# spacetelescope/subpixal

Measured on AMD Instinct MI355X. Metric: cutout cross-correlations/sec (64x64 px, upsample=10), higher is better.
Workload: dtype f32; 1 GPU; BASELINE.json configs[1]: 100000 64x64 Gaussian-spot cutout pairs per GPU, upsample=10, inputs resident in HBM; pairs_per_gpu=100000, tile=64, upsample=10, cc_type=CC, refine=default, parallelism=batch sharded over 1 GPU(s); gather of (dx,dy) to rank 0

## Files before the change

### subpixal_amd/csrc/spx_kernels.h

```cpp
#pragma once

namespace spx {

using rt::f32x2;
using rt::f32x4;
typedef f32x2 cf;

constexpr int kThreads = 256;

SPX_DEVICE int fresh_tid() { return rt::launder_lane(rt::thread_id()); }

enum { ST_OK = 0, ST_EDGE = 1, ST_NOMAX = 2, ST_OUTSIDE = 3, ST_WINDOW = 4, ST_FEWPTS = 5, ST_NONFINITE = 6, ST_SHAPE = 7 };
constexpr int kNoIndex = 0x7fffffff;
enum { CC_PLAIN = 0, CC_NCC = 1, CC_ZNCC = 2 };

constexpr int kNumPhases = 20;
template <int DBG> struct PhaseClock {
    unsigned long long last;
    unsigned long long acc[DBG == 100 ? kNumPhases : 1];
    SPX_DEVICE void start() {
        if constexpr (DBG == 100) {
            for (int i = 0; i < kNumPhases; ++i) acc[i] = 0;
            last = rt::clock_stamp();
        }
// ... 48 lines not shown
#pragma unroll
        for (int y = 0; y < 8; ++y) t[y] = v[y][x];
        fft8<DIR>(t);
#pragma unroll
        for (int y = 0; y < 8; ++y) v[y][x] = t[y];
    }
}
template <int DIR> SPX_DEVICE void fft8_x(cf (&v)[8][8]) {
#pragma unroll
    for (int y = 0; y < 8; ++y) fft8<DIR>(v[y]);
}

#ifndef SPX_CMUL_BATCH
#define SPX_CMUL_BATCH 1
#endif
template <bool CONJ> SPX_DEVICE void mul_row(cf (&v)[8][8], int y, cf w) {
    if constexpr (SPX_CMUL_BATCH) {
        rt::cmul8_ip<CONJ>(v[y][0], v[y][1], v[y][2], v[y][3], v[y][4], v[y][5], v[y][6], v[y][7], w);
    } else {
#pragma unroll
        for (int x = 0; x < 8; ++x) { if (CONJ) rt::cmulc_ip(v[y][x], w); else rt::cmul_ip(v[y][x], w); }
    }
}
template <bool CONJ> SPX_DEVICE void mul_col(cf (&v)[8][8], int x, cf w) {
    if constexpr (SPX_CMUL_BATCH) {
        rt::cmul8_ip<CONJ>(v[0][x], v[1][x], v[2][x], v[3][x], v[4][x], v[5][x], v[6][x], v[7][x], w);
    } else {
#pragma unroll
        for (int y = 0; y < 8; ++y) { if (CONJ) rt::cmulc_ip(v[y][x], w); else rt::cmul_ip(v[y][x], w); }
    }
}

template <int XS> SPX_DEVICE void transpose_tile(cf (&v)[8][8], float* xch, int lane) {
#pragma unroll
    for (int part = 0; part < 2; ++part) {
#pragma unroll
        for (int r = 0; r < 64; ++r)
            xch[r * XS + lane] = part ? v[r >> 3][r & 7].y : v[r >> 3][r & 7].x;
        rt::wave_sync();
#pragma unroll
        for (int r = 0; r < 64; ++r) {
            const float t = xch[lane * XS + r];
            if (part) v[r >> 3][r & 7].y = t; else v[r >> 3][r & 7].x = t;
        }
        rt::wave_sync();
    }
}

template <int XS> SPX_DEVICE void transpose_tile_v(cf (&v)[8][8], float* xch, int lane) {
#pragma unroll
    for (int part = 0; part < 2; ++part) {
#pragma unroll
        for (int r = 0; r < 64; ++r)
            xch[r * XS + lane] = part ? v[r >> 3][r & 7].y : v[r >> 3][r & 7].x;
        rt::wave_sync();
#pragma unroll
        for (int r = 0; r < 64; ++r) {
            const float t = rt::lds_read_f32(xch + lane * XS + r);
            if (part) v[r >> 3][r & 7].y = t; else v[r >> 3][r & 7].x = t;
        }
        rt::wave_sync();
    }
}

template <int XS> SPX_DEVICE void transpose_tile_w(cf (&v)[8][8], float* xch, int lane) {
    static_assert(XS >= 68 && (XS & 3) == 0, "32 complex slots per row plus the conflict padding");
    cf* buf = reinterpret_cast<cf*>(xch);
    cf t[64];
#pragma unroll
    for (int h = 0; h < 2; ++h) {
        if ((lane >> 5) == h) {
#pragma unroll
            for (int r = 0; r < 64; ++r) buf[r * (XS / 2) + (lane & 31)] = v[r >> 3][r & 7];
        }
        rt::wave_sync();
        const f32x4* row = reinterpret_cast<const f32x4*>(buf + lane * (XS / 2));
#pragma unroll
        for (int j = 0; j < 16; ++j) {
            const f32x4 q = row[j];
            t[32 * h + 2 * j] = cf{q[0], q[1]};
            t[32 * h + 2 * j + 1] = cf{q[2], q[3]};
        }
        rt::wave_sync();
    }
#pragma unroll
    for (int r = 0; r < 64; ++r) v[r >> 3][r & 7] = t[r];
}

#ifndef SPX_TRANSPOSE_VARIANT
#define SPX_TRANSPOSE_VARIANT 0
#endif
template <int XS> SPX_DEVICE void transpose_tile_sel(cf (&v)[8][8], float* xch, int lane) {
    if constexpr (SPX_TRANSPOSE_VARIANT == 1) transpose_tile_v<XS>(v, xch, lane);
    else if constexpr (SPX_TRANSPOSE_VARIANT == 2) transpose_tile_w<XS>(v, xch, lane);
    else transpose_tile<XS>(v, xch, lane);
}

SPX_DEVICE int plane_elem(int row, int col) { return row * 64 + (col ^ ((row & 7) << 3)); }
SPX_DEVICE int plane_slot(int n) { return n ^ (((n >> 4) & 7) << 1); }

template <int XS> SPX_DEVICE void transpose_tile_cplx(cf (&v)[8][8], float* xch, int lane) {
    constexpr int RS = 66;
    static_assert(32 * RS * 2 <= 64 * XS, "half a tile must fit the wave's exchange buffer");
    cf* buf = reinterpret_cast<cf*>(xch);
    cf t[64];
#pragma unroll
    for (int h = 0; h < 2; ++h) {
#pragma unroll
        for (int r = 0; r < 32; ++r) buf[r * RS + lane] = v[(32 * h + r) >> 3][(32 * h + r) & 7];
        rt::wave_sync();
        if ((lane >> 5) == h) {
            const f32x4* row = reinterpret_cast<const f32x4*>(buf + (lane & 31) * RS);
#pragma unroll
            for (int j = 0; j < 32; ++j) {
                const f32x4 q = row[j];
                t[2 * j] = cf{q[0], q[1]};
                t[2 * j + 1] = cf{q[2], q[3]};
            }
        }
        rt::wave_sync();
    }
#pragma unroll
    for (int r = 0; r < 64; ++r) v[r >> 3][r & 7] = t[r];
}

template <int C> struct Lds {
    static constexpr int P = 64 * C;
    static constexpr int T = 32 * C;
    static constexpr int NCLS = C * C;
    static constexpr int ZS = 72;
    static constexpr int XS = 68;
    static constexpr int PS = 64;
    static constexpr int TW_OFF = 0;
    static constexpr int SCR_OFF = TW_OFF + P * 8;
    static constexpr int R_OFF = SCR_OFF + 1024;
    static constexpr int ZBUF_BYTES = 2 * 64 * ZS * 4;
    static constexpr int XCH_WAVE_BYTES = 64 * XS * 4;
    static constexpr int XCH_BYTES = NCLS * XCH_WAVE_BYTES;
    static constexpr int PLANE_STRIDE_BYTES = XCH_WAVE_BYTES;
    static constexpr int FB_OFF = R_OFF + XCH_BYTES;
    static constexpr int cmax(int a, int b) { return a > b ? a : b; }
    static constexpr int fb_count(int W) { return W <= 16 ? NCLS : 1; }
    static constexpr int total(int W) {
        return cmax(R_OFF + cmax(ZBUF_BYTES, XCH_BYTES), FB_OFF + fb_count(W) * W * W * 4);
    }
};

constexpr int SCR_RED_F = 0;
constexpr int SCR_INT = 64;
constexpr int SCR_RED_D = 128;
constexpr int SCR_FIT = 256;
constexpr int SCR_STAT = 512;
constexpr int SCR_RED_D6 = 576;

SPX_DEVICE double wave_sum(double v) {
#pragma unroll
    for (int m = 32; m >= 1; m >>= 1) v += rt::shfl_xor(v, m);
    return v;
}

template <int NV> SPX_DEVICE void block_sum(unsigned char* lds_scr, double (&v)[NV]) {
    static_assert(NV <= 4 || NV == 6, "scratch slots exist for up to 4 values, or exactly 6");
    constexpr int ST = NV <= 4 ? 4 : 6;
    const int tid = rt::thread_id();
    double* part = reinterpret_cast<double*>(lds_scr + (NV <= 4 ? SCR_RED_D : SCR_RED_D6));
#pragma unroll
    for (int i = 0; i < NV; ++i) v[i] = wave_sum(v[i]);
    if ((tid & 63) == 0) {
#pragma unroll
        for (int i = 0; i < NV; ++i) part[(tid >> 6) * ST + i] = v[i];
    }
    rt::block_sync_lds();
#pragma unroll
    for (int i = 0; i < NV; ++i) {
        double s = 0.0;
        for (int w = 0; w < kThreads / 64; ++w) s += part[w * ST + i];
        v[i] = s;
    }
    rt::block_sync_lds();
}

SPX_DEVICE void block_sum2f(unsigned char* lds_scr, float& a, float& b) {
    const int tid = rt::thread_id();
#pragma unroll
    for (int m = 32; m >= 1; m >>= 1) {
        a += rt::shfl_xor(a, m);
        b += rt::shfl_xor(b, m);
    }
    float* part = reinterpret_cast<float*>(lds_scr + SCR_STAT);
    if ((tid & 63) == 0) { part[2 * (tid >> 6)] = a; part[2 * (tid >> 6) + 1] = b; }
    rt::block_sync_lds();
    a = (part[0] + part[2]) + (part[4] + part[6]);
    b = (part[1] + part[3]) + (part[5] + part[7]);
}

SPX_DEVICE bool better(float v, int i, float bv, int bi) {
    return (v > bv) || (v == bv && i < bi);
}
SPX_DEVICE float nan_as_inf(float v) { return v != v ? __builtin_inff() : v; }

template <int STEP> SPX_DEVICE void argmax_step(float& v, int& idx) {
    const float ov = rt::row_xchg<STEP>(v);
    const int oi = rt::row_xchg<STEP>(idx);
    if (better(ov, oi, v, idx)) { v = ov; idx = oi; }
}
SPX_DEVICE void wave_argmax(float& v, int& idx) {
    argmax_step<0>(v, idx);
    argmax_step<1>(v, idx);
    argmax_step<2>(v, idx);
    argmax_step<3>(v, idx);
    float bv = rt::read_lane(v, 0);
    int bi = rt::read_lane(idx, 0);
#pragma unroll
    for (int r = 1; r < 4; ++r) {
        const float ov = rt::read_lane(v, 16 * r);
        const int oi = rt::read_lane(idx, 16 * r);
        if (better(ov, oi, bv, bi)) { bv = ov; bi = oi; }
    }
    v = bv;
    idx = bi;
}

SPX_DEVICE void block_argmax(unsigned char* lds_scr, float& v, int& idx, int slot) {
    const int tid = rt::thread_id();
    wave_argmax(v, idx);
    float* rf = reinterpret_cast<float*>(lds_scr + SCR_RED_F) + 8 * slot;
    int* ri = reinterpret_cast<int*>(lds_scr + SCR_RED_F) + 8 * slot + 4;
    if ((tid & 63) == 0) { rf[tid >> 6] = v; ri[tid >> 6] = idx; }
    rt::block_sync_lds();
    v = rf[0];
    idx = ri[0];
    for (int w = 1; w < kThreads / 64; ++w)
        if (better(rf[w], ri[w], v, idx)) { v = rf[w]; idx = ri[w]; }
}

struct PeakResult {
    double x, y;
    int status;
};

SPX_DEVICE PeakResult quad_fit_finish(double s0, double sx, double sy, double sxy, double sxx,
                                      double syy, int x1, int y1, int imax, int jmax, int nx,
                                      int ny) {
    const double c10 = sx * (1.0 / 50.0), c01 = sy * (1.0 / 50.0), c11 = sxy * (1.0 / 100.0);
    const double c20 = (sxx - 2.0 * s0) * (1.0 / 70.0), c02 = (syy - 2.0 * s0) * (1.0 / 70.0);
    PeakResult r;
    const double det = 4.0 * c02 * c20 - c11 * c11;
    if (det <= 0.0 || ((c20 > 0.0 && c02 >= 0.0) || (c20 >= 0.0 && c02 > 0.0))) {
        r.x = x1 + 2.5;
        r.y = y1 + 2.5;
        r.status = ST_NOMAX;
        return r;
    }
    const double inv_det = 1.0 / det;
    const double xm = (x1 + 2) + (c01 * c11 - 2.0 * c02 * c10) * inv_det;
    const double ym = (y1 + 2) + (c10 * c11 - 2.0 * c01 * c20) * inv_det;
    if (xm > 0.0 && xm < nx - 1.0 && ym > 0.0 && ym < ny - 1.0) {
        r.x = xm;
        r.y = ym;
        r.status = ST_OK;
    } else {
        r.x = (double)imax;
        r.y = (double)jmax;
        r.status = ST_OUTSIDE;
    }
    return r;
}

SPX_DEVICE PeakResult quad_fit_5x5(const double* d, int x1, int y1, int imax, int jmax,
                                   int nx, int ny) {
    double s0 = 0, sx = 0, sy = 0, sxy = 0, sxx = 0, syy = 0;
    for (int j = 0; j < 5; ++j) {
        for (int i = 0; i < 5; ++i) {
            double v = d[j * 5 + i];
            double x = (double)(i - 2), y = (double)(j - 2);
            s0 += v;
            sx += x * v;
            sy += y * v;
            sxy += x * y * v;
            sxx += x * x * v;
            syy += y * y * v;
        }
    }
    return quad_fit_finish(s0, sx, sy, sxy, sxx, syy, x1, y1, imax, jmax, nx, ny);
}

SPX_DEVICE PeakResult quad_fit_wave(float v, int lane, int x1, int y1, int imax, int jmax,
                                    int nx, int ny) {
    lane = rt::launder_lane(lane);
    const int j = lane < 6 ? lane : 0;
    const int px = (j == 1 || j == 3) ? 1 : (j == 4 ? 2 : 0);
    const int py = (j == 2 || j == 3) ? 1 : (j == 5 ? 2 : 0);
    double xw[5], yw[5];
#pragma unroll
    for (int i = 0; i < 5; ++i) {
        const double c = (double)(i - 2);
        xw[i] = px == 0 ? 1.0 : (px == 1 ? c : c * c);
        yw[i] = py == 0 ? 1.0 : (py == 1 ? c : c * c);
    }
    double s = 0.0;
#pragma unroll
    for (int y = 0; y < 5; ++y) {
        double row = 0.0;
#pragma unroll
        for (int x = 0; x < 5; ++x) row += xw[x] * (double)rt::read_lane(v, 5 * y + x);
        s += yw[y] * row;
    }
    const double s0 = rt::read_lane(s, 0), sx = rt::read_lane(s, 1), sy = rt::read_lane(s, 2);
    const double sxy = rt::read_lane(s, 3), sxx = rt::read_lane(s, 4), syy = rt::read_lane(s, 5);
    return quad_fit_finish(s0, sx, sy, sxy, sxx, syy, x1, y1, imax, jmax, nx, ny);
}

SPX_DEVICE int64_t first_item(int64_t b, int64_t nwg) {
#ifdef SPX_LINEAR_WALK
    return b;
#endif
    if (nwg & 63) return b;
    const int64_t x = b & 7, j = b >> 3;
    return ((j >> 3) << 6) + (x << 3) + (j & 7);
}

template <int C> SPX_DEVICE void load_twiddles(unsigned char* lds, const cf* __restrict__ tw_g) {
    typedef Lds<C> L;
    cf* tw = reinterpret_cast<cf*>(lds + L::TW_OFF);
    for (int i = rt::thread_id(); i < L::P; i += kThreads) tw[i] = tw_g[i];
    rt::block_sync_lds();
}

SPX_DEVICE float warm_next_pair(const float* __restrict__ ref, const float* __restrict__ img) {
    const int tid = rt::thread_id();
    const float* p = (tid < 128) ? ref + tid * 32 : img + (tid - 128) * 32;
    return *p;
}

template <typename T> struct NormStatsT {
    T im_mean, im_rstd, ref_mean, ref_rstd;
    int active;
};

template <typename T> struct Quad { T v[4]; };
struct __attribute__((packed, aligned(4))) PackedF4 { float v[4]; };
struct __attribute__((packed, aligned(8))) PackedD2 { double v[2]; };
struct __attribute__((packed, aligned(4))) PackedF2 { float v[2]; };
SPX_DEVICE Quad<float> load_quad(const float* p) {
    const PackedF4 t = *reinterpret_cast<const PackedF4*>(p);
    return Quad<float>{{t.v[0], t.v[1], t.v[2], t.v[3]}};
}
SPX_DEVICE Quad<double> load_quad(const double* p) {
    const PackedD2 a = *reinterpret_cast<const PackedD2*>(p);
    const PackedD2 b = *reinterpret_cast<const PackedD2*>(p + 2);
    return Quad<double>{{a.v[0], a.v[1], b.v[0], b.v[1]}};
}
template <typename T> SPX_DEVICE float norm_im(T m, const NormStatsT<T>& ns) {
    if (m != (T)0) { m = m - ns.im_mean; m = m * ns.im_rstd; }
    return (float)m;
}
template <typename T> SPX_DEVICE float norm_ref(T r, const NormStatsT<T>& ns) {
    r = r - ns.ref_mean;
    return (float)(r * ns.ref_rstd);
}

template <typename TIn> struct ChunkLoad {
    Quad<TIn> r, t;
    int s;
    bool in;
};
template <typename TIn, bool NARROW, bool NX4 = false>
SPX_DEVICE ChunkLoad<TIn> chunk_issue(const TIn* __restrict__ ref, const TIn* __restrict__ img,
                                      int ny, int nx, int y, int x) {
    ChunkLoad<TIn> c;
    c.in = y < ny && x < nx;
    const int yy = y < ny ? y : ny - 1;
    if (NARROW) {
        c.s = 4 - nx;
        const TIn* rrow = ref + (int64_t)yy * nx;
        const TIn* mrow = img + (int64_t)(ny - 1 - yy) * nx;
#pragma unroll
        for (int k = 0; k < 4; ++k) {
            c.r.v[k] = k >= c.s ? rrow[k - c.s] : (TIn)0;
            c.t.v[k] = k < nx ? mrow[k] : (TIn)0;
        }
        c.in = c.in && x == 0;
        return c;
    }
    const int xx = x < nx ? x : 0;
    int s = xx + 4 - nx;
    s = (NX4 || s < 0) ? 0 : s;
    c.s = s;
    c.r = load_quad(ref + (int64_t)yy * nx + (xx - s));
    c.t = load_quad(img + (int64_t)(ny - 1 - yy) * nx + (nx - 4 - xx + s));
    return c;
}
template <typename T> SPX_DEVICE T quad_pick(const Quad<T>& q, int k) {
    const T lo = k & 1 ? q.v[1] : q.v[0], hi = k & 1 ? q.v[3] : q.v[2];
    return k & 2 ? hi : lo;
}
template <typename TIn>
SPX_DEVICE void chunk_unpack(const ChunkLoad<TIn>& c, const NormStatsT<TIn>& ns, float (&re)[4],
                             float (&im)[4]) {
#pragma unroll
    for (int e = 0; e < 4; ++e) {
        const bool ok = c.in && e + c.s < 4;
        const TIn ri = quad_pick(c.r, (e + c.s) & 3);
        const TIn mi = quad_pick(c.t, (3 - c.s - e) & 3);
        float r = (float)ri, m = (float)mi;
        if (ns.active) {
            m = norm_im(mi, ns);
            r = norm_ref(ri, ns);
        }
        re[e] = ok ? r : 0.0f;
        im[e] = ok ? m : 0.0f;
    }
}

template <int C, bool FOLD> struct StageGeom {
    static constexpr int ZS = FOLD ? 88 : 96;
    static constexpr int ROWS = FOLD ? 88 : 64;
    static constexpr int CHUNKS = (FOLD ? 88 : 64) / 4;
    static constexpr int PS12 = 12;
    static_assert(2 * ROWS * ZS * 4 <= Lds<C>::XCH_BYTES, "the staged input must fit the exchange region it shares");
    static SPX_DEVICE int perm(int q, int e) { return (4 * (q & 1) + e) * PS12 + (q >> 1); }
};

template <int C, bool FOLD = false, typename TIn = float, bool NARROW = false, bool NX4 = false>
SPX_DEVICE void stage_pair_rows(unsigned char* lds, const TIn* __restrict__ ref,
                           const TIn* __restrict__ img, int ny, int nx,
                           const NormStatsT<TIn>& ns, float (&ssq)[2]) {
    typedef Lds<C> L;
    typedef StageGeom<C, FOLD> G;
    float sr = 0.0f, sm = 0.0f;
    const int tid = fresh_tid();
    float* zre = reinterpret_cast<float*>(lds + L::R_OFF);
    float* zim = zre + G::ROWS * G::ZS;
    const bool aligned = ((reinterpret_cast<uintptr_t>(ref) | reinterpret_cast<uintptr_t>(img)) & 15) == 0;
    if constexpr (!FOLD && sizeof(TIn) == 4) if (ny == 64 && nx == 64 && aligned) {
        const f32x4* r4 = reinterpret_cast<const f32x4*>(ref);
        const f32x4* m4 = reinterpret_cast<const f32x4*>(img);
#pragma unroll
        for (int i = 0; i < 4; ++i) {
            const int idx = tid + i * kThreads;
            const int y = idx >> 4;
            f32x4 r = r4[idx];
            const f32x4 t = m4[(63 - y) * 16 + (15 - (idx & 15))];
            f32x4 m = f32x4{t[3], t[2], t[1], t[0]};
            if (ns.active) {
#pragma unroll
                for (int e = 0; e < 4; ++e) {
                    m[e] = norm_im(m[e], ns);
                    r[e] = norm_ref(r[e], ns);
                }
            }
#pragma unroll
            for (int e = 0; e < 4; ++e) {
                zre[y * G::ZS + G::perm(idx & 15, e)] = r[e];
                zim[y * G::ZS + G::perm(idx & 15, e)] = m[e];
                sr += r[e] * r[e];
                sm += m[e] * m[e];
            }
        }
        ssq[0] = sr;
        ssq[1] = sm;
        return;
    }
    constexpr int kIters = (G::ROWS * G::CHUNKS + kThreads - 1) / kThreads;
    ChunkLoad<TIn> ld[kIters];
#pragma unroll
    for (int i = 0; i < kIters; ++i) {
        const int idx = tid + i * kThreads;
        const int y = FOLD ? idx / G::CHUNKS : idx >> 4;
        const int x = (FOLD ? idx - y * G::CHUNKS : (idx & 15)) << 2;
        ld[i] = chunk_issue<TIn, NARROW, NX4>(ref, img, ny, nx, y, x);
    }
#pragma unroll
    for (int i = 0; i < kIters; ++i) {
        const int idx = tid + i * kThreads;
        if (FOLD && idx >= G::ROWS * G::CHUNKS) break;
        const int y = FOLD ? idx / G::CHUNKS : idx >> 4;
        const int x = (FOLD ? idx - y * G::CHUNKS : (idx & 15)) << 2;
        float rr[4], mm[4];
        chunk_unpack(ld[i], ns, rr, mm);
        if constexpr (FOLD) {
            *reinterpret_cast<f32x4*>(zre + y * G::ZS + x) = f32x4{rr[0], rr[1], rr[2], rr[3]};
            *reinterpret_cast<f32x4*>(zim + y * G::ZS + x) = f32x4{mm[0], mm[1], mm[2], mm[3]};
        } else {
#pragma unroll
            for (int e = 0; e < 4; ++e) {
                zre[y * G::ZS + G::perm(x >> 2, e)] = rr[e];
                zim[y * G::ZS + G::perm(x >> 2, e)] = mm[e];
            }
        }
#pragma unroll
        for (int e = 0; e < 4; ++e) { sr += rr[e] * rr[e]; sm += mm[e] * mm[e]; }
    }
    ssq[0] = sr;
    ssq[1] = sm;
}
template <int C, bool FOLD = false, typename TIn = float>
SPX_DEVICE void stage_pair(unsigned char* lds, const TIn* __restrict__ ref,
                           const TIn* __restrict__ img, int ny, int nx,
                           const NormStatsT<TIn>& ns, float (&ssq)[2]) {
    if (nx < 4) stage_pair_rows<C, FOLD, TIn, true>(lds, ref, img, ny, nx, ns, ssq);
    else if ((nx & 3) == 0) stage_pair_rows<C, FOLD, TIn, false, true>(lds, ref, img, ny, nx, ns, ssq);
    else stage_pair_rows<C, FOLD, TIn, false>(lds, ref, img, ny, nx, ns, ssq);
}

SPX_DEVICE float balance_from_ssq(float s0, float s1) {
    if (!(s0 > 0.0f) || !(s1 > 0.0f)) return 1.0f;
    const int e0 = (int)((__builtin_bit_cast(unsigned, s0) >> 23) & 0xffu);
    const int e1 = (int)((__builtin_bit_cast(unsigned, s1) >> 23) & 0xffu);
    int e = (e0 - e1) >> 1;
    e = e < -100 ? -100 : (e > 100 ? 100 : e);
    return __builtin_bit_cast(float, (unsigned)(127 + e) << 23);
}
SPX_DEVICE float balance_factor(unsigned char* lds_scr, float (&ssq)[2]) {
    block_sum2f(lds_scr, ssq[0], ssq[1]);
    return balance_from_ssq(ssq[0], ssq[1]);
}

SPX_DEVICE int plane_col(int row, int col) { return col ^ (((row & 1) << 4) | ((row & 2) << 2)); }

#ifndef SPX_DISP5_CPLXT
#define SPX_DISP5_CPLXT 0
#endif
#ifndef SPX_FUSED_TW
#define SPX_FUSED_TW 0
#endif
template <int K> SPX_DEVICE f32x2 quad_pair(f32x4 q) {
    if constexpr (K < 2) return f32x2{q[0], q[1]}; else return f32x2{q[2], q[3]};
}
template <int K, bool CONJ> SPX_DEVICE cf soa_cmul_k(f32x4 re4, f32x4 im4, cf w) {
    return rt::bcast_fma_rot<(K & 1), CONJ>(quad_pair<K>(im4), w, rt::bcast_mul<(K & 1), CONJ>(quad_pair<K>(re4), w));
}
template <bool CONJ> SPX_DEVICE cf soa_cmul(int k, f32x4 re4, f32x4 im4, cf w) {
    switch (k & 3) {
        case 0: return soa_cmul_k<0, CONJ>(re4, im4, w);
        case 1: return soa_cmul_k<1, CONJ>(re4, im4, w);
        case 2: return soa_cmul_k<2, CONJ>(re4, im4, w);
        default: return soa_cmul_k<3, CONJ>(re4, im4, w);
    }
}
template <int K> SPX_DEVICE cf soa_cmul2_k(f32x4 re4, f32x4 im4, cf w, cf bw) {
    return rt::bcast_fma_rot<(K & 1), false>(quad_pair<K>(im4), bw, rt::bcast_mul<(K & 1), false>(quad_pair<K>(re4), w));
}
SPX_DEVICE cf soa_cmul2(int k, f32x4 re4, f32x4 im4, cf w, cf bw) {
    switch (k & 3) {
        case 0: return soa_cmul2_k<0>(re4, im4, w, bw);
        case 1: return soa_cmul2_k<1>(re4, im4, w, bw);
        case 2: return soa_cmul2_k<2>(re4, im4, w, bw);
        default: return soa_cmul2_k<3>(re4, im4, w, bw);
    }
}

template <int XS, bool CONJ, bool W0_ONE>
SPX_DEVICE void transpose_tile_tw(cf (&v)[8][8], float* xch, int lane, const cf (&w)[8]) {
    f32x4 re4[16], im4[16];
#pragma unroll
    for (int part = 0; part < 2; ++part) {
#pragma unroll
        for (int r = 0; r < 64; ++r)
            xch[r * XS + lane] = part ? v[r >> 3][r & 7].y : v[r >> 3][r & 7].x;
        rt::wave_sync();
        const f32x4* row = reinterpret_cast<const f32x4*>(xch + lane * XS);
#pragma unroll
        for (int j = 0; j < 16; ++j) { if (part) im4[j] = row[j]; else re4[j] = row[j]; }
        rt::wave_sync();
    }
#pragma unroll
    for (int r = 0; r < 64; ++r) {
        const int b = r & 7;
        if (W0_ONE && b == 0) v[r >> 3][b] = cf{re4[r >> 2][r & 3], im4[r >> 2][r & 3]};
        else v[r >> 3][b] = soa_cmul<CONJ>(r, re4[r >> 2], im4[r >> 2], w[b]);
    }
}

template <typename G, int CY, int CX>
SPX_DEVICE void load_tile_class(cf (&v)[8][8], const float* zre, const float* zim, const cf* tw, float bal,
                                int l1, int l0) {
    constexpr int NK = 7 * (CY + CX) + 1;
    cf W[NK], BW[NK];
#pragma unroll
    for (int k = 1; k < NK; ++k) { W[k] = tw[8 * k]; BW[k] = cf{bal * W[k].x, bal * W[k].y}; }
#pragma unroll
    for (int y1 = 0; y1 < 8; ++y1) {
        const f32x4* pr = reinterpret_cast<const f32x4*>(zre + (l1 + 8 * y1) * G::ZS + l0 * G::PS12);
        const f32x4* pi = reinterpret_cast<const f32x4*>(zim + (l1 + 8 * y1) * G::ZS + l0 * G::PS12);
        const f32x4 r0 = pr[0], r1 = pr[1], i0 = pi[0], i1 = pi[1];
#pragma unroll
        for (int x1 = 0; x1 < 8; ++x1) {
            const int k = CY * y1 + CX * x1;
            const f32x4 rq = x1 < 4 ? r0 : r1, iq = x1 < 4 ? i0 : i1;
            if (k == 0) v[y1][x1] = cf{rq[x1 & 3], bal * iq[x1 & 3]};
            else v[y1][x1] = soa_cmul2(x1, rq, iq, W[k], BW[k]);
        }
    }
}

template <typename L, int CY, int CX>
SPX_DEVICE void store_plane_class(const cf (&v)[8][8], float* plane, const cf* tw, int l1, int l0) {
    constexpr int NK = 7 * (CY + CX) + 1;
    cf W[NK];
#pragma unroll
    for (int k = 1; k < NK; ++k) W[k] = tw[8 * k];
#pragma unroll
    for (int x1 = 0; x1 < 8; ++x1)
#pragma unroll
        for (int y1 = 0; y1 < 8; ++y1) {
            const cf a = v[y1][x1];
            const int k = CY * y1 + CX * x1;
            const int row = l1 + 8 * y1;
            plane[row * L::PS + plane_col(row, l0 + 8 * x1)] = k == 0 ? a.y : a.y * W[k].x - a.x * W[k].y;
        }
}
// ... 345 lines not shown
#pragma unroll
        for (int b = 0; b < WB; ++b)
#pragma unroll
            for (int i = 0; i < 4; ++i) {
                ft.ky[b][i] = kty[b * 64 * 4 + i];
                ft.kx[b][i] = ktx[b * 64 * 4 + i];
            }
    }
}

template <int C, int WB, typename R>
SPX_DEVICE void fine_window(unsigned char* lds, const FineTables<WB, R>& ft,
                            int ny, int nx, int qyc, int qxc, int rot = 0) {
    typedef Lds<C> L;
    typedef typename R::S S;
    typedef typename R::V4 V4;
    static_assert(C == 2, "");
    constexpr int W = 16 * WB;
    const int tid = fresh_tid();
    const int wave = ((tid >> 6) + rot) & (C * C - 1), lane = tid & 63;
    const int cy = wave / C, cx = wave % C;
    const int lk = lane >> 4, lj = lane & 15;
    const float* plane = reinterpret_cast<const float*>(lds + L::R_OFF + wave * L::PLANE_STRIDE_BYTES);
    float* fbuf = reinterpret_cast<float*>(lds + L::FB_OFF);
    const int lyc = conv_index(ny, qyc), lxc = conv_index(nx, qxc);

    V4 acc[WB][4];
#pragma unroll
    for (int ab = 0; ab < WB; ++ab)
#pragma unroll
        for (int t = 0; t < 4; ++t) acc[ab][t] = R::zero();
    int col[4];
#pragma unroll
    for (int t = 0; t < 4; ++t) col[t] = (lxc + 16 * t + lj - 32) & 63;

    float afrag[16][4];
#pragma unroll
    for (int step = 0; step < 16; ++step) {
        const int row = (lyc + 4 * step + lk - 32) & 63;
#pragma unroll
        for (int t = 0; t < 4; ++t) afrag[step][t] = plane[row * L::PS + plane_col(row, col[t])];
    }
#pragma unroll
    for (int s4 = 0; s4 < 4; ++s4) {
        V4 kb[WB];
#pragma unroll
        for (int ab = 0; ab < WB; ++ab) kb[ab] = ft.y(ab, s4);
#pragma unroll
        for (int e = 0; e < 4; ++e) {
            const int step = 4 * s4 + e;
            const int m = lyc + 4 * step + lk - 32;
            const S sgn = (cy && ((m >> 6) & 1)) ? (S)-1 : (S)1;
#pragma unroll
            for (int t = 0; t < 4; ++t) {
#pragma unroll
                for (int ab = 0; ab < WB; ++ab)
                    acc[ab][t] = R::mma((S)afrag[step][t], sgn * kb[ab][e], acc[ab][t]);
            }
        }
    }
    const S scale = (S)0.5 / (S)(L::P * L::P);
    auto put = [&](int bb, int ab, const V4& fv, int c) {
#pragma unroll
        for (int r = 0; r < 4; ++r) {
            const int b = bb * 16 + R::drow(lk, r), a = ab * 16 + lj;
            const float val = (float)(fv[r] * scale);
            if constexpr (L::fb_count(W) == C * C) fbuf[wave * W * W + b * W + a] = val;
            else { if (c == 0) fbuf[b * W + a] = val; else fbuf[b * W + a] += val; }
        }
    };
    V4 f[WB][WB];
#pragma unroll
    for (int bb = 0; bb < WB; ++bb)
#pragma unroll
        for (int ab = 0; ab < WB; ++ab) f[bb][ab] = R::zero();
#pragma unroll
    for (int t = 0; t < 4; ++t) {
        V4 ka[WB];
#pragma unroll
        for (int bb = 0; bb < WB; ++bb) ka[bb] = ft.x(bb, t);
#pragma unroll
        for (int r = 0; r < 4; ++r) {
            const int m = lxc + 16 * t + R::drow(lk, r) - 32;
            const S sgn = (cx && ((m >> 6) & 1)) ? (S)-1 : (S)1;
#pragma unroll
            for (int bb = 0; bb < WB; ++bb)
#pragma unroll
                for (int ab = 0; ab < WB; ++ab)
                    f[bb][ab] = R::mma(sgn * ka[bb][r], acc[ab][t][r], f[bb][ab]);
        }
    }
    if constexpr (L::fb_count(W) == C * C) {
#pragma unroll
        for (int bb = 0; bb < WB; ++bb)
#pragma unroll
            for (int ab = 0; ab < WB; ++ab) put(bb, ab, f[bb][ab], 0);
        rt::block_sync_lds();
    } else {
        for (int c = 0; c < C * C; ++c) {
            if (wave == c) {
#pragma unroll
                for (int bb = 0; bb < WB; ++bb)
#pragma unroll
                    for (int ab = 0; ab < WB; ++ab) put(bb, ab, f[bb][ab], c);
            }
            rt::block_sync_lds();
        }
    }
}

template <int C>
SPX_DEVICE void load_afrag(const unsigned char* lds, float (&afrag)[16][4], int rot) {
    typedef Lds<C> L;
    const int tid = fresh_tid();
    const int wave = ((tid >> 6) + rot) & (C * C - 1), lane = tid & 63;
    const int lk = lane >> 4, lj = lane & 15;
    const float* plane = reinterpret_cast<const float*>(lds + L::R_OFF + wave * L::PLANE_STRIDE_BYTES);
#pragma unroll
    for (int step = 0; step < 16; ++step) {
        const int row = 4 * step + lk;
#pragma unroll
        for (int t = 0; t < 4; ++t) afrag[step][t] = plane[row * L::PS + plane_col(row, 16 * t + lj)];
    }
}

template <int WB> struct RolledTables {
    float y[WB][16];
    float x[WB][16];
};
template <int C, int WB>
SPX_DEVICE void load_rolled_tables(RolledTables<WB>& rt_, const float* __restrict__ ktab, int ny, int nx,
                                   int qyc, int qxc, int rot) {
    const int tid = fresh_tid();
    const int wave = ((tid >> 6) + rot) & (C * C - 1), lane = tid & 63;
    const int cy = wave / C, cx = wave % C;
    const int lk = lane >> 4, lj = lane & 15;
    constexpr int kBlk = 128 * 16;
    const float* sec = rt::launder(ktab) + 2 * 2 * WB * 64 * 16;
    const int dy = conv_index(ny, qyc) - 32, dx = conv_index(nx, qxc) - 32;
    const float* ty = sec + (cy * 2 + ((dy >> 6) & 1)) * WB * kBlk + (lk - (dy & 63) + 64) * 16 + lj;
    const float* tx = sec + (cx * 2 + ((dx >> 6) & 1)) * WB * kBlk + (4 * lk - (dx & 63) + 64) * 16 + lj;
#pragma unroll
    for (int b = 0; b < WB; ++b)
#pragma unroll
        for (int step = 0; step < 16; ++step) rt_.y[b][step] = ty[b * kBlk + 64 * step];
#pragma unroll
    for (int b = 0; b < WB; ++b)
#pragma unroll
        for (int t = 0; t < 4; ++t)
#pragma unroll
            for (int r = 0; r < 4; ++r) rt_.x[b][4 * t + r] = tx[b * kBlk + 16 * (16 * t + r)];
}

template <int C, int WB>
SPX_DEVICE void fine_window_rolled(unsigned char* lds, const float (&afrag)[16][4], const RolledTables<WB>& kt,
                                   int rot) {
    typedef Lds<C> L;
    typedef RefineF32 R;
    typedef R::V4 V4;
    static_assert(C == 2, "");
    constexpr int W = 16 * WB;
    const int tid = fresh_tid();
    const int wave = ((tid >> 6) + rot) & (C * C - 1), lane = tid & 63;
    const int lk = lane >> 4, lj = lane & 15;
    float* fbuf = reinterpret_cast<float*>(lds + L::FB_OFF);

    V4 acc[WB][4];
#pragma unroll
    for (int ab = 0; ab < WB; ++ab)
#pragma unroll
        for (int t = 0; t < 4; ++t) acc[ab][t] = R::zero();
#pragma unroll
    for (int step = 0; step < 16; ++step)
#pragma unroll
        for (int t = 0; t < 4; ++t)
#pragma unroll
            for (int ab = 0; ab < WB; ++ab) acc[ab][t] = R::mma(afrag[step][t], kt.y[ab][step], acc[ab][t]);
    const float scale = 0.5f / (float)(L::P * L::P);
    V4 f[WB][WB];
#pragma unroll
    for (int bb = 0; bb < WB; ++bb)
#pragma unroll
        for (int ab = 0; ab < WB; ++ab) f[bb][ab] = R::zero();
#pragma unroll
    for (int t = 0; t < 4; ++t)
#pragma unroll
        for (int r = 0; r < 4; ++r)
#pragma unroll
            for (int bb = 0; bb < WB; ++bb)
#pragma unroll
                for (int ab = 0; ab < WB; ++ab) f[bb][ab] = R::mma(kt.x[bb][4 * t + r], acc[ab][t][r], f[bb][ab]);
    auto put = [&](int bb, int ab, const V4& fv, int c) {
#pragma unroll
        for (int r = 0; r < 4; ++r) {
            const int b = bb * 16 + R::drow(lk, r), a = ab * 16 + lj;
            const float val = fv[r] * scale;
            if constexpr (L::fb_count(W) == C * C) fbuf[wave * W * W + b * W + a] = val;
            else { if (c == 0) fbuf[b * W + a] = val; else fbuf[b * W + a] += val; }
        }
    };
    if constexpr (L::fb_count(W) == C * C) {
#pragma unroll
        for (int bb = 0; bb < WB; ++bb)
#pragma unroll
            for (int ab = 0; ab < WB; ++ab) put(bb, ab, f[bb][ab], 0);
        rt::block_sync_lds();
    } else {
        for (int c = 0; c < C * C; ++c) {
            if (wave == c) {
#pragma unroll
                for (int bb = 0; bb < WB; ++bb)
#pragma unroll
                    for (int ab = 0; ab < WB; ++ab) put(bb, ab, f[bb][ab], c);
            }
            rt::block_sync_lds();
        }
    }
}

template <int C, int W>
SPX_DEVICE float fine_value(const unsigned char* lds, int b, int a) {
    typedef Lds<C> L;
    const float* fbuf = reinterpret_cast<const float*>(lds + L::FB_OFF);
    if constexpr (L::fb_count(W) == C * C) {
        float acc = fbuf[b * W + a];
#pragma unroll
        for (int c = 1; c < C * C; ++c) acc += fbuf[c * W * W + b * W + a];
        return acc;
    } else {
        return fbuf[b * W + a];
    }
}

template <int C>
SPX_DEVICE void coarse_argmax_fold(const unsigned char* lds, int ny, int nx, float& bv, int& bi) {
    typedef Lds<C> L;
    static_assert(C == 2, "");
    const int tid = fresh_tid();
    const int loy = (ny - 1) / 2, lox = (nx - 1) / 2;
    const int mx4 = (tid & 15) << 2;
    int qxa[4], qxb[4];
#pragma unroll
    for (int e = 0; e < 4; ++e) {
        const int mx = mx4 + e;
        qxa[e] = mx >= lox ? (nx - 1) + lox - mx : -1;
        qxb[e] = (nx - 1) + lox - mx - 64;
    }
    float m = -__builtin_inff();
    int best = kNoIndex;
#pragma unroll
    for (int i = 0; i < 4; ++i) {
        const int my = (tid >> 4) + 16 * i;
        const int qya = my >= loy ? (ny - 1) + loy - my : -1;
        const int qyb = (ny - 1) + loy - my - 64;
        f32x4 d[C * C];
#pragma unroll
        for (int c = 0; c < C * C; ++c)
            d[c] = *reinterpret_cast<const f32x4*>(lds + L::R_OFF + c * L::PLANE_STRIDE_BYTES +
                                                   (my * L::PS + plane_col(my, mx4)) * 4);
#pragma unroll
        for (int e = 0; e < 4; ++e) {
            const float up = d[0][e] + d[1][e], um = d[0][e] - d[1][e];
            const float tp = d[2][e] + d[3][e], tm = d[2][e] - d[3][e];
            const float vaa = up + tp, vab = um + tm, vba = up - tp, vbb = um - tm;
            if (qya >= 0 && qxa[e] >= 0 && better(vaa, qya * nx + qxa[e], m, best)) { m = vaa; best = qya * nx + qxa[e]; }
            if (qya >= 0 && qxb[e] >= 0 && better(vab, qya * nx + qxb[e], m, best)) { m = vab; best = qya * nx + qxb[e]; }
            if (qyb >= 0 && qxa[e] >= 0 && better(vba, qyb * nx + qxa[e], m, best)) { m = vba; best = qyb * nx + qxa[e]; }
            if (qyb >= 0 && qxb[e] >= 0 && better(vbb, qyb * nx + qxb[e], m, best)) { m = vbb; best = qyb * nx + qxb[e]; }
        }
    }
    bv = m;
    bi = best;
}

template <int C, bool FOLD = false>
SPX_DEVICE void coarse_argmax(const unsigned char* lds, int ny, int nx, float& bv, int& bi) {
    typedef Lds<C> L;
    static_assert(C == 2, "");
    if constexpr (FOLD) { coarse_argmax_fold<C>(lds, ny, nx, bv, bi); return; }
    const int tid = fresh_tid();
    const int loy = (ny - 1) / 2, lox = (nx - 1) / 2;
    const float ninf = -__builtin_inff();
    const int mx4 = (tid & 15) << 2;
    int qx[4];
    float fx[4];
#pragma unroll
    for (int e = 0; e < 4; ++e) {
        const int mx = mx4 + e;
        const bool wrap = mx < lox;
        qx[e] = (nx - 1) + lox - mx - (wrap ? 64 : 0);
        fx[e] = wrap ? -1.0f : 1.0f;
    }
    float val[4][4];
    int rowbase[4];
    float m = ninf;
#pragma unroll
    for (int i = 0; i < 4; ++i) {
        const int my = (tid >> 4) + 16 * i;
        const bool wrap = my < loy;
        const int qy = (ny - 1) + loy - my - (wrap ? 64 : 0);
        const float fy = wrap ? -1.0f : 1.0f;
        rowbase[i] = qy * nx;
        f32x4 d[C * C];
#pragma unroll
        for (int c = 0; c < C * C; ++c)
            d[c] = *reinterpret_cast<const f32x4*>(lds + L::R_OFF + c * L::PLANE_STRIDE_BYTES +
                                                   (my * L::PS + plane_col(my, mx4)) * 4);
#pragma unroll
        for (int e = 0; e < 4; ++e) {
            const float u = __builtin_fmaf(fx[e], d[1][e], d[0][e]);
            const float t = __builtin_fmaf(fx[e], d[3][e], d[2][e]);
            const float v = __builtin_fmaf(fy, t, u);
            val[i][e] = (qy >= 0 && qx[e] >= 0) ? v : ninf;
            m = __builtin_fmaxf(m, val[i][e]);
        }
    }
    int best = 0x7fffffff;
#pragma unroll
    for (int i = 0; i < 4; ++i)
#pragma unroll
        for (int e = 0; e < 4; ++e) {
            const int idx = (val[i][e] == m) ? rowbase[i] + qx[e] : 0x7fffffff;
            best = idx < best ? idx : best;
        }
    bv = m;
    bi = best;
}

template <typename ValFn>
SPX_DEVICE PeakResult peak_fit_wave0(unsigned char* lds_scr, int imax, int jmax, int NX, int NY,
                                     ValFn val, int fit_wave = 0) {
    const int tid = rt::thread_id() - 64 * fit_wave;
    PeakResult r;
    r.x = (double)imax; r.y = (double)jmax; r.status = ST_EDGE;
    if (imax == 0 || jmax == 0) return r;
    if (tid < 0 || tid >= 64) return r;
    int x1 = imax - 2, y1 = jmax - 2;
    if (x1 > NX - 5) x1 = NX - 5;
    if (y1 > NY - 5) y1 = NY - 5;
    if (x1 < 0) x1 = 0;
    if (y1 < 0) y1 = 0;
    const int k = tid < 25 ? tid : 24;
    const float v = val(x1 + k % 5, y1 + k / 5);
    return quad_fit_wave(v, tid, x1, y1, imax, jmax, NX, NY);
}

template <int C, int WB, int DBG = 0, bool FOLD = false, typename TIn = float, typename R = RefineF32>
SPX_DEVICE void pair_body(const TIn* __restrict__ ref, const TIn* __restrict__ img,
                          int ny, int nx, int U, int cc_type, const cf* __restrict__ tw_g,
                          const float* __restrict__ ktab, double* __restrict__ out,
                          int* __restrict__ status, unsigned char* lds, PhaseClock<DBG>& clk,
                          const TIn* __restrict__ next_ref, const TIn* __restrict__ next_img,
                          float& warm, int fit_wave, double inv_u) {
    typedef Lds<C> L;
    ny = rt::launder_uniform(ny);
    nx = rt::launder_uniform(nx);
    U = rt::launder_uniform(U);
    const int tid = fresh_tid();
    unsigned char* scr = lds + L::SCR_OFF;
    const NormStatsT<TIn> ns = norm_stats(scr, ref, img, 1, 0, ny, nx, cc_type);
    float ssq[2];
    rt::consume(warm);
    stage_pair<C, FOLD, TIn>(lds, ref, img, ny, nx, ns, ssq);
    const float bal = balance_factor(scr, ssq);
    const float oscale = 0.5f / ((float)(L::P * L::P) * bal);
    clk.tick(0);
    if constexpr (DBG == 1) return;
    const int rot = (C * C - fit_wave) & (C * C - 1);
    if (cc_planes<C, DBG, FOLD>(lds, bal, clk, rot)) return;
    if constexpr (DBG == 10) return;
    constexpr bool kRolled = WB == 1 && R::kRolled;
    FineTables<(WB > 0 ? WB : 1), R> ft;
    float afrag[kRolled ? 16 : 1][4];
    if constexpr (kRolled) load_afrag<C>(lds, afrag, rot);
    else if constexpr (WB > 0) load_fine_tables<C, WB, R>(ft, ktab, rot);
    if constexpr (sizeof(TIn) == 4 && !kRolled) if (next_ref) warm = warm_next_pair(next_ref, next_img);

    float bv;
    int bi;
    coarse_argmax<C, FOLD>(lds, ny, nx, bv, bi);
    block_argmax(scr, bv, bi, 0);
    const bool nonfinite = bi == kNoIndex;
    if (nonfinite) bi = 0;
    int qyc = bi / nx, qxc = bi - (bi / nx) * nx;
    clk.tick(11);
    if constexpr (DBG == 11) { if (tid == 0) out[0] = (double)bi; return; }

    PeakResult pk;
    if (nonfinite) {
        pk.x = 0.0; pk.y = 0.0; pk.status = ST_NONFINITE;
    } else if constexpr (WB == 0) {
        pk = peak_fit_wave0(scr, qxc, qyc, nx, ny, [&](int x, int y) {
            return window_value<C>(lds, ny, nx, y, x, oscale);
        }, fit_wave);
    } else {
        constexpr int W = 16 * (WB > 0 ? WB : 1);
        const int NX = U * nx, NY = U * ny;
        int imax = 0, jmax = 0;
        bool inside = false;
        for (int iter = 0; iter < 4; ++iter) {
            if constexpr (kRolled) {
                RolledTables<(WB > 0 ? WB : 1)> kt;
                load_rolled_tables<C, (WB > 0 ? WB : 1)>(kt, ktab, ny, nx, qyc, qxc, rot);
                if constexpr (sizeof(TIn) == 4) if (iter == 0 && next_ref) warm = warm_next_pair(next_ref, next_img);
                fine_window_rolled<C, (WB > 0 ? WB : 1)>(lds, afrag, kt, rot);
            } else {
                fine_window<C, (WB > 0 ? WB : 1), R>(lds, ft, ny, nx, qyc, qxc, rot);
            }
            clk.tick(12);
            if constexpr (DBG == 12) { if (tid == 0) out[0] = (double)fine_value<C, W>(lds, 0, 0); return; }
            const int fx0 = U * qxc - W / 2, fy0 = U * qyc - W / 2;
            float fv = -__builtin_inff();
            int fi = 0x7fffffff;
#pragma unroll 4
            for (int i = (tid & 63); i < W * W; i += 64) {
                const int b = i / W, a = i % W;
                const int idx = a * W + b;
                const int gy = fy0 + a, gx = fx0 + b;
                const float val = fine_value<C, W>(lds, b, a);
                const bool in = gy >= 0 && gy < NY && gx >= 0 && gx < NX;
                if (in && better(val, idx, fv, fi)) { fv = val; fi = idx; }
            }
            wave_argmax(fv, fi);
            clk.tick(13);
            if constexpr (DBG == 13) { if (tid == 0) out[0] = (double)fi; return; }
            if (fi == kNoIndex) { imax = jmax = -1; break; }
            const int a = fi / W, b = fi % W;
            jmax = fy0 + a;
            imax = fx0 + b;
            int x1 = imax - 2, y1 = jmax - 2;
            if (x1 > NX - 5) x1 = NX - 5;
            if (y1 > NY - 5) y1 = NY - 5;
            if (x1 < 0) x1 = 0;
            if (y1 < 0) y1 = 0;
            const bool okx = (x1 >= fx0 && x1 + 4 < fx0 + W) || imax == 0;
            const bool oky = (y1 >= fy0 && y1 + 4 < fy0 + W) || jmax == 0;
            if (okx && oky) { inside = true; break; }
            if (!okx) qxc += (b < W / 2) ? -1 : 1;
            if (!oky) qyc += (a < W / 2) ? -1 : 1;
            qxc = qxc < 0 ? 0 : (qxc > nx ? nx : qxc);
            qyc = qyc < 0 ? 0 : (qyc > ny ? ny : qyc);
            rt::block_sync_lds();
        }
        clk.tick(16);
        if (inside) {
            const int fx0 = U * qxc - W / 2, fy0 = U * qyc - W / 2;
            pk = peak_fit_wave0(scr, imax, jmax, NX, NY, [&](int x, int y) {
                return fine_value<C, W>(lds, x - fx0, y - fy0);
            }, fit_wave);
        } else if (imax < 0) {
            pk.x = 0.0; pk.y = 0.0; pk.status = ST_NONFINITE;
        } else {
            pk.x = (double)imax; pk.y = (double)jmax; pk.status = ST_WINDOW;
        }
    }
    clk.tick(17);
    if (tid == 64 * fit_wave) {
        out[0] = pk.x * inv_u - (double)((nx - 1) / 2);
        out[1] = pk.y * inv_u - (double)((ny - 1) / 2);
        if (status) status[0] = pk.status;
    }
    clk.tick(14);
}

template <int C, int WB, int DBG = 0, bool FOLD = false, typename TIn = float, typename R = RefineF32>
SPX_TKERNEL(256) void pair_kernel(const TIn* __restrict__ ref, const TIn* __restrict__ img,
                                  int64_t nbatch, int ny, int nx, int U, int cc_type,
                                  const cf* __restrict__ tw_g, const float* __restrict__ ktab,
                                  double* __restrict__ out, int* __restrict__ status) {
    SPX_DYN_LDS(lds);
    load_twiddles<C>(lds, tw_g);
    PhaseClock<DBG> clk;
    clk.start();
    const int64_t stride = (int64_t)ny * nx;
    const bool full = !FOLD && sizeof(TIn) == 4 && ny == 64 && nx == 64 &&
        ((reinterpret_cast<uintptr_t>(ref) | reinterpret_cast<uintptr_t>(img)) & 15) == 0;
    const int64_t step = rt::grid_size();
    float warm = 0.0f;
    int fit_wave = (int)(rt::block_id() & 3);
    const double inv_u = rt::read_lane(1.0 / (double)U, 0);
    for (int64_t p = first_item(rt::block_id(), step); p < nbatch; p += step) {
        const bool more = full && (p + step < nbatch);
        pair_body<C, WB, DBG, FOLD, TIn, R>(ref + p * stride, img + p * stride, ny, nx, U, cc_type, tw_g, ktab,
                              out + 2 * p, status ? status + p : nullptr, lds, clk,
                              more ? ref + (p + step) * stride : nullptr,
                              more ? img + (p + step) * stride : nullptr, warm, fit_wave, inv_u);
        fit_wave = (fit_wave + 1) & 3;
        if constexpr (WB == 0) rt::block_sync_lds();
        clk.tick(15);
    }
    if constexpr (DBG == 100)
        clk.flush(reinterpret_cast<unsigned long long*>(status + nbatch));
}

template <int C>
SPX_DEVICE void interlace_window_fold(const unsigned char* lds, int ny, int nx, float out_scale,
                                      float* __restrict__ icc, int ox, int oy, float& bv, int& bi) {
    typedef Lds<C> L;
    static_assert(C == 2, "");
    const int tid = fresh_tid();
    const int loy = (ny - 1) / 2, lox = (nx - 1) / 2;
    const int NX = 2 * nx;
    const int mx4 = (tid & 15) << 2;
    int gxa[4], gxb[4];
#pragma unroll
    for (int e = 0; e < 4; ++e) {
        const int mx = mx4 + e;
        const int qb = (nx - 1) + lox - mx - 64;
        gxa[e] = mx >= lox ? 2 * ((nx - 1) + lox - mx) + ox : -1;
        gxb[e] = qb >= 0 ? 2 * qb + ox : -1;
    }
    float m = bv;
    int best = bi;
#pragma unroll
    for (int i = 0; i < 4; ++i) {
        const int my = (tid >> 4) + 16 * i;
        const int qb = (ny - 1) + loy - my - 64;
        const int rowa = my >= loy ? (2 * ((ny - 1) + loy - my) + oy) * NX : -1;
        const int rowb = qb >= 0 ? (2 * qb + oy) * NX : -1;
        f32x4 d[C * C];
#pragma unroll
        for (int c = 0; c < C * C; ++c)
            d[c] = *reinterpret_cast<const f32x4*>(lds + L::R_OFF + c * L::PLANE_STRIDE_BYTES +
                                                   (my * L::PS + plane_col(my, mx4)) * 4);
#pragma unroll
        for (int e = 0; e < 4; ++e) {
            const float up = d[0][e] + d[1][e], um = d[0][e] - d[1][e];
            const float tp = d[2][e] + d[3][e], tm = d[2][e] - d[3][e];
            const float vaa = (up + tp) * out_scale, vab = (um + tm) * out_scale;
            const float vba = (up - tp) * out_scale, vbb = (um - tm) * out_scale;
            auto put = [&](int row, int gx, float v) {
                if (row >= 0 && gx >= 0) {
                    icc[row + gx] = v;
                    v = nan_as_inf(v);
                    if (better(v, row + gx, m, best)) { m = v; best = row + gx; }
                }
            };
            put(rowa, gxa[e], vaa);
            put(rowa, gxb[e], vab);
            put(rowb, gxa[e], vba);
            put(rowb, gxb[e], vbb);
        }
    }
    bv = m;
    bi = best;
}

template <int C, bool FOLD = false>
SPX_DEVICE void interlace_window(const unsigned char* lds, int ny, int nx, float out_scale,
                                 float* __restrict__ icc, int ox, int oy, float& bv, int& bi) {
    typedef Lds<C> L;
    static_assert(C == 2, "");
    if constexpr (FOLD) { interlace_window_fold<C>(lds, ny, nx, out_scale, icc, ox, oy, bv, bi); return; }
    const int tid = fresh_tid();
    const int loy = (ny - 1) / 2, lox = (nx - 1) / 2;
    const int NX = 2 * nx;
    const float ninf = -__builtin_inff();
    const int mx4 = (tid & 15) << 2;
    int gx[4];
    float fx[4];
#pragma unroll
    for (int e = 0; e < 4; ++e) {
        const int mx = mx4 + e;
        const bool wrap = mx < lox;
        const int qx = (nx - 1) + lox - mx - (wrap ? 64 : 0);
        gx[e] = qx >= 0 ? 2 * qx + ox : -1;
        fx[e] = wrap ? -1.0f : 1.0f;
    }
    float val[4][4];
    int rowbase[4];
    float m = ninf;
#pragma unroll
    for (int i = 0; i < 4; ++i) {
        const int my = (tid >> 4) + 16 * i;
        const bool wrap = my < loy;
        const int qy = (ny - 1) + loy - my - (wrap ? 64 : 0);
        const float fy = wrap ? -1.0f : 1.0f;
        rowbase[i] = qy >= 0 ? (2 * qy + oy) * NX : -1;
        f32x4 d[C * C];
#pragma unroll
        for (int c = 0; c < C * C; ++c)
            d[c] = *reinterpret_cast<const f32x4*>(lds + L::R_OFF + c * L::PLANE_STRIDE_BYTES +
                                                   (my * L::PS + plane_col(my, mx4)) * 4);
#pragma unroll
        for (int e = 0; e < 4; ++e) {
            const float u = __builtin_fmaf(fx[e], d[1][e], d[0][e]);
            const float t = __builtin_fmaf(fx[e], d[3][e], d[2][e]);
            const float v = __builtin_fmaf(fy, t, u) * out_scale;
            const bool ok = rowbase[i] >= 0 && gx[e] >= 0;
            if (ok) icc[rowbase[i] + gx[e]] = v;
            val[i][e] = ok ? nan_as_inf(v) : ninf;
            m = __builtin_fmaxf(m, val[i][e]);
        }
    }
    int best = 0x7fffffff;
#pragma unroll
    for (int i = 0; i < 4; ++i)
#pragma unroll
        for (int e = 0; e < 4; ++e) {
            const int idx = (val[i][e] == m) ? rowbase[i] + gx[e] : 0x7fffffff;
            best = idx < best ? idx : best;
        }
    if (better(m, best, bv, bi)) { bv = m; bi = best; }
}

template <int C, bool FOLD = false, typename TIn = float>
SPX_DEVICE void disp5_body(const TIn* __restrict__ ref, const TIn* __restrict__ im4,
                           int ny, int nx, int cc_type, const cf* __restrict__ tw_g,
                           float* __restrict__ icc, double* __restrict__ out,
                           int* __restrict__ status, unsigned char* lds) {
    typedef Lds<C> L;
    unsigned char* scr = lds + L::SCR_OFF;
    const int64_t stride = (int64_t)ny * nx;
    NormStatsT<TIn> ns = norm_stats(scr, ref, im4, 4, stride, ny, nx, cc_type);
    ns.im_mean = rt::read_lane(ns.im_mean, 0);
    ns.im_rstd = rt::read_lane(ns.im_rstd, 0);
    ns.ref_mean = rt::read_lane(ns.ref_mean, 0);
    ns.ref_rstd = rt::read_lane(ns.ref_rstd, 0);
    ns.active = rt::read_lane(ns.active, 0);

    float bv = -__builtin_inff();
    int bi = 0x7fffffff;
    const int NX = 2 * nx, NY = 2 * ny;
    for (int q = 0; q < 4; ++q) {
        const int ox = q & 1, oy = q >> 1;
        float ssq[2];
        stage_pair<C, FOLD, TIn>(lds, ref, im4 + q * stride, ny, nx, ns, ssq);
        const float bal = balance_factor(scr, ssq);
        const float oscale = 0.5f / ((float)(L::P * L::P) * bal);
        PhaseClock<0> noclk;
        cc_planes<C, 0, FOLD, SPX_DISP5_CPLXT>(lds, bal, noclk);
        interlace_window<C, FOLD>(lds, ny, nx, oscale, icc, ox, oy, bv, bi);
        rt::block_sync_lds();
    }
    rt::block_sync();
    block_argmax(scr, bv, bi, 0);
    const bool nonfinite = !(bv < __builtin_inff());
    const int jmax = bi / NX, imax = bi % NX;
    PeakResult pk;
// ... 72 lines not shown
```

Before: 26.56 million cross-correlations/s.

## Stage next pair's tiles into LDS during current pair's fine-window MMA

During the first refinement iteration, the kernel now issues global loads for the next cutout pair and interleaves writing them into the LDS staging region between the fine-window matrix steps. It also accumulates the per-wave sum-of-squares partials into a scratch slot, so the next pair can skip norm_stats and stage_pair. This hides load and staging latency behind MMA work and replaces the old cache-warming prefetch. The cost is higher register pressure from holding the loads. It also relies on the staged LDS region not being overwritten by the remaining refinement iterations and argmax, which is a correctness risk. It only applies to plain CC with 64x64 aligned f32 input.

```diff
diff --git a/subpixal_amd/csrc/spx_kernels.h b/subpixal_amd/csrc/spx_kernels.h
--- a/subpixal_amd/csrc/spx_kernels.h
+++ b/subpixal_amd/csrc/spx_kernels.h
@@ -224,6 +224,7 @@
 constexpr int SCR_FIT = 256;
 constexpr int SCR_STAT = 512;
 constexpr int SCR_RED_D6 = 576;
+constexpr int SCR_AHEAD = 768;
 
 SPX_DEVICE double wave_sum(double v) {
 #pragma unroll
@@ -494,6 +495,38 @@
     static SPX_DEVICE int perm(int q, int e) { return (4 * (q & 1) + e) * PS12 + (q >> 1); }
 };
 
+struct FullTileLoads { f32x4 r[4], t[4]; };
+SPX_DEVICE void stage_full_issue(FullTileLoads& ld, const float* __restrict__ ref, const float* __restrict__ img,
+                                 int tid) {
+    const f32x4* r4 = reinterpret_cast<const f32x4*>(ref);
+    const f32x4* m4 = reinterpret_cast<const f32x4*>(img);
+#pragma unroll
+    for (int i = 0; i < 4; ++i) {
+        const int idx = tid + i * kThreads;
+        const int y = idx >> 4;
+        ld.r[i] = r4[idx];
+        ld.t[i] = m4[(63 - y) * 16 + (15 - (idx & 15))];
+    }
+}
+template <int C>
+SPX_DEVICE void stage_full_piece(unsigned char* lds, const FullTileLoads& ld, int i, int e, int tid,
+                                 const NormStatsT<float>& ns, float& sr, float& sm) {
+    typedef StageGeom<C, false> G;
+    float* zre = reinterpret_cast<float*>(lds + Lds<C>::R_OFF);
+    float* zim = zre + G::ROWS * G::ZS;
+    const int idx = tid + i * kThreads;
+    const int y = idx >> 4;
+    float r = ld.r[i][e], m = ld.t[i][3 - e];
+    if (ns.active) {
+        m = norm_im(m, ns);
+        r = norm_ref(r, ns);
+    }
+    zre[y * G::ZS + G::perm(idx & 15, e)] = r;
+    zim[y * G::ZS + G::perm(idx & 15, e)] = m;
+    sr += r * r;
+    sm += m * m;
+}
+
 template <int C, bool FOLD = false, typename TIn = float, bool NARROW = false, bool NX4 = false>
 SPX_DEVICE void stage_pair_rows(unsigned char* lds, const TIn* __restrict__ ref,
                            const TIn* __restrict__ img, int ny, int nx,
@@ -506,30 +539,12 @@
     float* zim = zre + G::ROWS * G::ZS;
     const bool aligned = ((reinterpret_cast<uintptr_t>(ref) | reinterpret_cast<uintptr_t>(img)) & 15) == 0;
     if constexpr (!FOLD && sizeof(TIn) == 4) if (ny == 64 && nx == 64 && aligned) {
-        const f32x4* r4 = reinterpret_cast<const f32x4*>(ref);
-        const f32x4* m4 = reinterpret_cast<const f32x4*>(img);
-#pragma unroll
-        for (int i = 0; i < 4; ++i) {
-            const int idx = tid + i * kThreads;
-            const int y = idx >> 4;
-            f32x4 r = r4[idx];
-            const f32x4 t = m4[(63 - y) * 16 + (15 - (idx & 15))];
-            f32x4 m = f32x4{t[3], t[2], t[1], t[0]};
-            if (ns.active) {
-#pragma unroll
-                for (int e = 0; e < 4; ++e) {
-                    m[e] = norm_im(m[e], ns);
-                    r[e] = norm_ref(r[e], ns);
-                }
-            }
-#pragma unroll
-            for (int e = 0; e < 4; ++e) {
-                zre[y * G::ZS + G::perm(idx & 15, e)] = r[e];
-                zim[y * G::ZS + G::perm(idx & 15, e)] = m[e];
-                sr += r[e] * r[e];
-                sm += m[e] * m[e];
-            }
-        }
+        FullTileLoads ld;
+        stage_full_issue(ld, ref, img, tid);
+#pragma unroll
+        for (int i = 0; i < 4; ++i)
+#pragma unroll
+            for (int e = 0; e < 4; ++e) stage_full_piece<C>(lds, ld, i, e, tid, ns, sr, sm);
         ssq[0] = sr;
         ssq[1] = sm;
         return;
@@ -1181,9 +1196,10 @@
             for (int r = 0; r < 4; ++r) rt_.x[b][4 * t + r] = tx[b * kBlk + 16 * (16 * t + r)];
 }
 
-template <int C, int WB>
+struct NoMidWork { SPX_DEVICE void operator()(int) const {} };
+template <int C, int WB, typename Mid = NoMidWork>
 SPX_DEVICE void fine_window_rolled(unsigned char* lds, const float (&afrag)[16][4], const RolledTables<WB>& kt,
-                                   int rot) {
+                                   int rot, Mid mid = Mid()) {
     typedef Lds<C> L;
     typedef RefineF32 R;
     typedef R::V4 V4;
@@ -1214,11 +1230,13 @@
 #pragma unroll
     for (int t = 0; t < 4; ++t)
 #pragma unroll
-        for (int r = 0; r < 4; ++r)
+        for (int r = 0; r < 4; ++r) {
 #pragma unroll
             for (int bb = 0; bb < WB; ++bb)
 #pragma unroll
                 for (int ab = 0; ab < WB; ++ab) f[bb][ab] = R::mma(kt.x[bb][4 * t + r], acc[ab][t][r], f[bb][ab]);
+            mid(4 * t + r);
+        }
     auto put = [&](int bb, int ab, const V4& fv, int c) {
 #pragma unroll
         for (int r = 0; r < 4; ++r) {
@@ -1380,25 +1398,38 @@
                           const float* __restrict__ ktab, double* __restrict__ out,
                           int* __restrict__ status, unsigned char* lds, PhaseClock<DBG>& clk,
                           const TIn* __restrict__ next_ref, const TIn* __restrict__ next_img,
-                          float& warm, int fit_wave, double inv_u) {
+                          float& warm, bool& staged, int fit_wave, double inv_u) {
     typedef Lds<C> L;
     ny = rt::launder_uniform(ny);
     nx = rt::launder_uniform(nx);
     U = rt::launder_uniform(U);
     const int tid = fresh_tid();
     unsigned char* scr = lds + L::SCR_OFF;
-    const NormStatsT<TIn> ns = norm_stats(scr, ref, img, 1, 0, ny, nx, cc_type);
-    float ssq[2];
-    rt::consume(warm);
-    stage_pair<C, FOLD, TIn>(lds, ref, img, ny, nx, ns, ssq);
-    const float bal = balance_factor(scr, ssq);
+    constexpr bool kRolled = WB == 1 && R::kRolled;
+    constexpr bool kAhead = kRolled && !FOLD && sizeof(TIn) == 4 && (DBG == 0 || DBG == 100);
+    bool was_staged = false;
+    if constexpr (kAhead) was_staged = staged;
+    staged = false;
+    float bal;
+    if (was_staged) {
+        const float* part = reinterpret_cast<const float*>(scr + SCR_AHEAD);
+        const float s0 = (part[0] + part[2]) + (part[4] + part[6]);
+        const float s1 = (part[1] + part[3]) + (part[5] + part[7]);
+        bal = balance_from_ssq(s0, s1);
+        clk.tick(19);
+    } else {
+        const NormStatsT<TIn> ns = norm_stats(scr, ref, img, 1, 0, ny, nx, cc_type);
+        float ssq[2];
+        rt::consume(warm);
+        stage_pair<C, FOLD, TIn>(lds, ref, img, ny, nx, ns, ssq);
+        bal = balance_factor(scr, ssq);
+        clk.tick(0);
+    }
     const float oscale = 0.5f / ((float)(L::P * L::P) * bal);
-    clk.tick(0);
     if constexpr (DBG == 1) return;
     const int rot = (C * C - fit_wave) & (C * C - 1);
     if (cc_planes<C, DBG, FOLD>(lds, bal, clk, rot)) return;
     if constexpr (DBG == 10) return;
-    constexpr bool kRolled = WB == 1 && R::kRolled;
     FineTables<(WB > 0 ? WB : 1), R> ft;
     float afrag[kRolled ? 16 : 1][4];
     if constexpr (kRolled) load_afrag<C>(lds, afrag, rot);
@@ -1431,8 +1462,48 @@
             if constexpr (kRolled) {
                 RolledTables<(WB > 0 ? WB : 1)> kt;
                 load_rolled_tables<C, (WB > 0 ? WB : 1)>(kt, ktab, ny, nx, qyc, qxc, rot);
-                if constexpr (sizeof(TIn) == 4) if (iter == 0 && next_ref) warm = warm_next_pair(next_ref, next_img);
-                fine_window_rolled<C, (WB > 0 ? WB : 1)>(lds, afrag, kt, rot);
+                bool ahead = false;
+                if constexpr (kAhead) ahead = iter == 0 && next_ref && cc_type == CC_PLAIN;
+                if (ahead) {
+                    if constexpr (kAhead) {
+                        FullTileLoads nl;
+                        const int atid = fresh_tid();
+                        stage_full_issue(nl, reinterpret_cast<const float*>(next_ref),
+                                         reinterpret_cast<const float*>(next_img), atid);
+                        rt::sched_fence();
+                        NormStatsT<float> nns;
+                        nns.active = 0;
+                        nns.im_mean = 0; nns.im_rstd = 1; nns.ref_mean = 0; nns.ref_rstd = 1;
+                        float sr = 0.0f, sm = 0.0f;
+                        auto finish = [&]() {
+#pragma unroll
+                            for (int m = 32; m >= 1; m >>= 1) {
+                                sr += rt::shfl_xor(sr, m);
+                                sm += rt::shfl_xor(sm, m);
+                            }
+                            float* part = reinterpret_cast<float*>(scr + SCR_AHEAD);
+                            if ((atid & 63) == 0) { part[2 * (atid >> 6)] = sr; part[2 * (atid >> 6) + 1] = sm; }
+                        };
+                        auto commit = [&](int k) {
+                            if constexpr (DBG == 100) {
+                                if (k != 15) return;
+                                clk.tick(12);
+#pragma unroll
+                                for (int j = 0; j < 16; ++j) stage_full_piece<C>(lds, nl, j >> 2, j & 3, atid, nns, sr, sm);
+                                finish();
+                                clk.tick(18);
+                            } else {
+                                stage_full_piece<C>(lds, nl, k >> 2, k & 3, atid, nns, sr, sm);
+                                if (k == 15) finish();
+                            }
+                        };
+                        fine_window_rolled<C, (WB > 0 ? WB : 1)>(lds, afrag, kt, rot, commit);
+                        staged = true;
+                    }
+                } else {
+                    if constexpr (sizeof(TIn) == 4) if (iter == 0 && next_ref) warm = warm_next_pair(next_ref, next_img);
+                    fine_window_rolled<C, (WB > 0 ? WB : 1)>(lds, afrag, kt, rot);
+                }
             } else {
                 fine_window<C, (WB > 0 ? WB : 1), R>(lds, ft, ny, nx, qyc, qxc, rot);
             }
@@ -1506,6 +1577,7 @@
         ((reinterpret_cast<uintptr_t>(ref) | reinterpret_cast<uintptr_t>(img)) & 15) == 0;
     const int64_t step = rt::grid_size();
     float warm = 0.0f;
+    bool staged = false;
     int fit_wave = (int)(rt::block_id() & 3);
     const double inv_u = rt::read_lane(1.0 / (double)U, 0);
     for (int64_t p = first_item(rt::block_id(), step); p < nbatch; p += step) {
@@ -1513,7 +1585,7 @@
         pair_body<C, WB, DBG, FOLD, TIn, R>(ref + p * stride, img + p * stride, ny, nx, U, cc_type, tw_g, ktab,
                               out + 2 * p, status ? status + p : nullptr, lds, clk,
                               more ? ref + (p + step) * stride : nullptr,
-                              more ? img + (p + step) * stride : nullptr, warm, fit_wave, inv_u);
+                              more ? img + (p + step) * stride : nullptr, warm, staged, fit_wave, inv_u);
         fit_wave = (fit_wave + 1) & 3;
         if constexpr (WB == 0) rt::block_sync_lds();
         clk.tick(15);
```

Result: faster. 27.30 million cross-correlations/s (median of 6 runs) (+2.8%).
